# dhg14n9/Light-path-tracer

Hardware: AMD Instinct MI355X
Metric: Mrays/s (higher is better)
Workload: dtype f32

## Files before the change

### include/ltrace.h

```cpp
#ifndef LTRACE_H
#define LTRACE_H

#include <stddef.h>
#include <stdint.h>

#ifdef __cplusplus
extern "C" {
#endif

#define LT_VERSION 200

#define LT_OK 0
#define LT_ERR_INVALID_ARG (-1)
#define LT_ERR_HIP (-2)
#define LT_ERR_NO_DEVICE (-3)
#define LT_ERR_UNSUPPORTED (-4)

#define LT_METRIC_SCHWARZSCHILD 0
#define LT_METRIC_KERR 1

#define LT_INTEGRATOR_DP45 0
#define LT_INTEGRATOR_RK4 1
#define LT_INTEGRATOR_DP45_EXACT 2

// ... 81 lines not shown
                        int8_t *out_status, uint32_t *out_rhs_evals);

int lt_trace_batch_kerr(double M, double a, double r_obs, const double *alphas, const double *thetas,
                        double theta_obs, double lambda_max, const uint8_t *axis_refines,
                        int integrator, int precision, int schedule, int64_t n, double *out_fa,
                        int64_t *out_w, int8_t *out_status, uint32_t *out_rhs_evals);

int lt_trace_batch_kerr_general_probe(double M, double a, double r_obs, const double *alphas, const double *thetas,
                                      double theta_obs, double lambda_max, const uint8_t *axis_refines, int precision,
                                      int64_t n, double *out_fa, int64_t *out_w, int8_t *out_status,
                                      uint32_t *out_rhs_evals);

int lt_set_eq_streak(int on);

int lt_set_unit_streak(int on);

int lt_sincos_q1_probe(uint32_t bits_lo, uint32_t bits_hi, uint64_t out[4], float band[2]);

int lt_kerr_rhs_probe(double M, double a, const double *states, const double *p_phi, int64_t n,
                      int precision, double *out);

int lt_kerr_rhs_form_probe(double M, double a, const double *states, const double *p_phi, int64_t n, int precision,
                           int form, double *out);

int lt_kerr_step_probe(double M, double a, const double *states, const double *p_phi, const uint8_t *refine,
                       const double *h, int64_t n, int precision, int form, double *out_states, double *out_min_r,
                       double *out_max_d, double *out_cs);


int lt_dp45_attempt_probe(double M, double a, double r_obs, double lambda_max, const double *states, const double *p_phi,
// ... 388 lines not shown
```

### light-path-tracer_amd/csrc/lt_api.hip

```cpp
#include "../../include/ltrace.h"
#include "lt_kernels.hpp"
#include "lt_disk.hpp"
#include "lt_disk_images.hpp"
#include "lt_hit_time.hpp"
#include "lt_hotspot.hpp"
#include "lt_polarization.hpp"
#include "lt_aa.hpp"
#include "lt_aa_adaptive.hpp"
#include "lt_hotspot_aa.hpp"
#include "lt_diskmap.hpp"
#include "lt_spectrum.hpp"
#include "lt_visibility.hpp"
#include "lt_visibility_stokes.hpp"
#ifdef LT_PROBES
#include "lt_probe.hpp"
#endif
#include "lt_dense.hpp"

#include <algorithm>
#include <array>
#include <atomic>
#include <cmath>
#include <cstdarg>
#include <cstdio>
// ... 1 lines not shown
#include <cstdlib>
#include <mutex>
#include <type_traits>
#include <utility>
#include <vector>

#ifndef LT_BUILD_ID
#define LT_BUILD_ID "unversioned"
#endif

using namespace lt;

namespace lt {
extern template __global__ void k_kerr_direct<float, Rk4<float>>(KerrConsts<float>, const typename Vec4<float>::type *__restrict__,
                                                                 typename Vec4<float>::type *__restrict__, typename Vec4<float>::type *__restrict__,
                                                                 int64_t, uint32_t, uint4 *__restrict__, uint64_t *__restrict__, unsigned long long *__restrict__);
}

static thread_local char g_err[512] = "";

static int fail(int code, const char *fmt, ...)
{
    va_list ap;
    va_start(ap, fmt);
    vsnprintf(g_err, sizeof(g_err), fmt, ap);
    va_end(ap);
    return code;
}

#define HIP_TRY(expr)                                                                             \
    do {                                                                                          \
// ... 58 lines not shown
    Grow dev;
    Grow dense;
    Grow blocks;
    Grow disk_img;
    Grow disk_time;
    Grow disk_mom;
    Grow hotspot;
    Grow spectrum;
    Grow visibility;
    std::vector<int32_t> blocks_host;
    EventQuad own{};
    bool own_ok = false;
    std::vector<EventQuad> aa_events;
    Grow aa_list;
    Grow aa_scratch;
};

struct Ctx {
    std::vector<StreamSlot *> slots;
    std::vector<EventQuad> pending;
    std::vector<EventQuad> pool;
};

static int slot_events(StreamSlot *sl)
{
    if (sl->own_ok) return LT_OK;
    int made = 0;
    for (auto &e : sl->own.e) {
        if (hipEventCreate(&e) != hipSuccess) break;
        ++made;
    }
    if (made != (int)(sizeof(sl->own.e) / sizeof(sl->own.e[0]))) {
        for (int j = 0; j < made; ++j) (void)hipEventDestroy(sl->own.e[j]);
        return fail(LT_ERR_HIP, "hipEventCreate failed");
    }
    sl->own_ok = true;
    return LT_OK;
}

static std::mutex g_mu;
static Ctx g_ctx[64];
struct MultiStream { int dev, idx; hipStream_t s; };
static std::vector<MultiStream> g_multi_streams;

static int cur_ctx(Ctx **out)
{
    int dev = 0;
    HIP_TRY(hipGetDevice(&dev));
    if (dev < 0 || dev >= 64) return fail(LT_ERR_INVALID_ARG, "device index %d out of range", dev);
    *out = &g_ctx[dev];
    return LT_OK;
// ... 29 lines not shown
    return LT_OK;
}

static void release(Grow &g)
{
    if (g.p) (void)hipFree(g.p);
    g.p = nullptr;
    g.bytes = 0;
}

static void destroy_slot(StreamSlot *sl)
{
    for (Grow *g : {&sl->ws, &sl->dev, &sl->dense, &sl->blocks, &sl->disk_img, &sl->disk_time, &sl->disk_mom, &sl->hotspot, &sl->spectrum, &sl->visibility, &sl->aa_list, &sl->aa_scratch}) release(*g);
    if (sl->own_ok) for (auto &e : sl->own.e) (void)hipEventDestroy(e);
    for (auto &q : sl->aa_events) for (auto &e : q.e) (void)hipEventDestroy(e);
    delete sl;
}

constexpr size_t WS_CTRL_BYTES = 256 + (size_t)STAT_SLOTS * 8 * sizeof(unsigned long long);
struct Workspace {
    unsigned long long *head, *partials;
    char *records;
    size_t n_q;
    template <typename T> typename Vec4<T>::type *ic() const { return (typename Vec4<T>::type *)records; }
    template <typename T> typename Vec4<T>::type *fin0() const { return ic<T>() + n_q; }
    template <typename T> typename Vec4<T>::type *fin1() const { return ic<T>() + 2 * n_q; }
};

template <typename F> static auto with_precision(int precision, F f) { return precision == 32 ? f(float{}) : f(double{}); }
static size_t elem_size(int precision) { return precision == 32 ? sizeof(float) : sizeof(double); }

static int get_workspace(hipStream_t stream, size_t n_q, size_t elem, Workspace *w, StreamSlot **slot = nullptr,
                         IcKey *held = nullptr)
{
    StreamSlot *sl;
    int rc = get_slot(stream, &sl);
    if (rc) return rc;
    if (slot) *slot = sl;
    {
        std::lock_guard<std::mutex> lk(g_mu);
        if (held) *held = sl->ic_key;
        sl->ic_key.valid = false;
    }
    size_t vec = 4 * elem;
    const void *before = sl->ws.p;
    const size_t bytes_before = sl->ws.bytes;
    if ((rc = grow(sl->ws, WS_CTRL_BYTES + 3 * n_q * vec, stream))) return rc;
    if (held && sl->ws.bytes != bytes_before) held->valid = false;
    if (sl->ws.p != before) HIP_TRY(hipMemsetAsync(sl->ws.p, 0, WS_CTRL_BYTES, stream));
    char *base = (char *)sl->ws.p;
    w->head = (unsigned long long *)base;
    w->partials = (unsigned long long *)(base + 256);
    w->records = base + WS_CTRL_BYTES;
    w->n_q = n_q;
    return LT_OK;
}

struct Carver {
    size_t off = 0;
    size_t take(size_t bytes) { size_t o = off; off += (bytes + 255) & ~(size_t)255; return o; }
};

static int env_int(const char *name, int dflt)
{
    const char *e = getenv(name);
    return e ? atoi(e) : dflt;
// ... 27 lines not shown
static bool unit_streak_enabled()
{
    int v = g_unit_streak.load(std::memory_order_relaxed);
    if (v < 0) {
        v = env_int("LT_UNIT_STREAK", 1) != 0;
        int unset = -1;
        if (!g_unit_streak.compare_exchange_strong(unset, v)) v = unset;
    }
    return v != 0;
}
extern "C" int lt_set_unit_streak(int on)
{
    const int before = unit_streak_enabled();
    g_unit_streak.store(on != 0);
    return before;
}

static uint64_t g_ic_hits = 0, g_ic_misses = 0;
extern "C" void lt_ic_reuse_counts(uint64_t *hits, uint64_t *misses)
{
    std::lock_guard<std::mutex> lk(g_mu);
    if (hits) *hits = g_ic_hits;
    if (misses) *misses = g_ic_misses;
}

static int cu_count(int *out)
{
    static int cached[64];
    int dev = 0;
    HIP_TRY(hipGetDevice(&dev));
// ... 349 lines not shown
    return t;
}

template <typename T, typename Go> static int with_integrator(const lt_opts &o, int long_rk4, Go go)
{
    const bool exact = o.integrator == LT_INTEGRATOR_DP45_EXACT;
    const bool dp45 = o.integrator == LT_INTEGRATOR_DP45 || exact;
    if (dp45 && sizeof(T) != 8) return fail(LT_ERR_UNSUPPORTED, "DP45 needs precision 64");
    if constexpr (sizeof(T) == 8) {
        if (exact) return go(IntegTag<Dp45<T, true>>{}, long_rk4 / 3);
        if (dp45) return go(IntegTag<Dp45<T>>{}, long_rk4 / 3);
    }
    return go(IntegTag<Rk4<T>>{}, long_rk4);
}

template <typename T, typename Kernels, typename Launch>
static int launch_direct(const lt_opts &o, const Workspace &w, int64_t n_q, hipStream_t s, int block, Launch launch)
{
    const DirectTuning &tune = direct_tuning();
    return with_integrator<T>(o, tune.long_iters, [&](auto integ, int long_it) -> int {
        constexpr auto kernel = Kernels::template kernel<typename decltype(integ)::type>;
        unsigned grid = (unsigned)((n_q + block - 1) / block);
        unsigned long long *head = nullptr;
        const int slots = tune.persist && block == 64 ? resident_slots<kernel>() : 0;
        if (slots > 0 && (unsigned)slots < grid) { grid = (unsigned)slots; head = w.head; }
        if (head) HIP_TRY(hipMemsetAsync(head, 0, sizeof(unsigned long long), s));
        launch(kernel, grid, (uint32_t)long_it, head);
        HIP_TRY(hipGetLastError());
        return LT_OK;
    });
}

template <typename T>
static int launch_integrate(const MetricConsts &mc, const lt_opts &o, double lambda_max, const Workspace &w,
                            int64_t n_q, hipStream_t s, uint64_t *kstats)
{
    int rc;
    unsigned grid = (unsigned)((n_q + 255) / 256);
    if (mc.kind == LT_METRIC_SCHWARZSCHILD) {
        SchwConsts<T> k = make_schw<T>(mc, o.phi_max, o.h_max);
        k_schw_rk4_direct<T><<<grid, 256, 0, s>>>(k, w.ic<T>(), w.fin0<T>(), w.fin1<T>(), n_q);
    } else {
        KerrConsts<T> k = make_kerr<T>(mc, lambda_max, o.h_max);
        StampDump sd;
        if (o.schedule == LT_SCHED_DIRECT) {
            static const int k2_block = [] { int b = env_int("LT_K2_BLOCK", 64);
                                             return (b == 64 || b == 128 || b == 256) ? b : 64; }();
            if ((rc = sd.begin((size_t)(n_q / 64)))) return rc;
            rc = launch_direct<T, PlainKernels<T>>(o, w, n_q, s, k2_block, [&](auto kernel, unsigned kgrid, uint32_t long_iters, unsigned long long *head) {
                kernel<<<kgrid, k2_block, 0, s>>>(k, w.ic<T>(), w.fin0<T>(), w.fin1<T>(), n_q, long_iters, sd.dev, kstats, head);
            });
            if (rc) return rc;
        } else {
            int cus;
            if ((rc = cu_count(&cus))) return rc;
            static const int bpc = env_int("LT_Q_BPC", sizeof(T) == 4 ? 8 : 3);
            static const int chunk = env_int("LT_Q_CHUNK", 64);
            static const int refill_min = env_int("LT_Q_REFILL", 4);
            static const int long_steps = env_int("LT_Q_LONG", 600);
            unsigned qgrid = (unsigned)(cus * bpc);
            if (qgrid > grid) qgrid = grid;
            rc = with_integrator<T>(o, long_steps, [&](auto integ, int long_it) -> int {
                HIP_TRY(hipMemsetAsync(w.head, 0, sizeof(unsigned long long), s));
                if (int brc = sd.begin((size_t)qgrid * 4)) return brc;
                k_kerr_queue<T, typename decltype(integ)::type><<<qgrid, 256, 0, s>>>(k, w.ic<T>(), w.fin0<T>(), w.fin1<T>(), (uint64_t)n_q, w.head,
// ... 101 lines not shown
            return launch_integrate_disk<decltype(t)>(mc, o, lambda_max, w, n_q, s, kstats, *disk, recs);
        });
    return with_precision(o.precision, [&](auto t) { return launch_integrate<decltype(t)>(mc, o, lambda_max, w, n_q, s, kstats); });
}

template <typename Launch> static void launch_epilogue_rows(const CamConsts &c, const lt_opts &o, const FrameOut &fo, Launch launch)
{
    const bool has_bg = fo.bg != nullptr && (fo.rgb || fo.rgba);
    const dim3 ge((unsigned)((c.W + EPILOGUE_BLOCK - 1) / EPILOGUE_BLOCK), (unsigned)c.rows_local);
    with_precision(o.precision, [&](auto t) {
        if (has_bg) launch(t, std::true_type{}, ge);
        else launch(t, std::false_type{}, ge);
    });
}

static int launch_epilogue_frame(const CamConsts &c, const MetricConsts &mc, const lt_opts &o, const Workspace &w,
                                 const FrameOut &fo, uint64_t *d_stats, hipStream_t s)
{
    if (o.bg_sampling == LT_BG_LDS_TILES && fo.bg && (fo.rgb || fo.rgba)) {
        const unsigned gp = (unsigned)((int64_t)((c.W + 15) / 16) * ((c.rows_local + 15) / 16));
        with_precision(o.precision, [&](auto t) {
            using T = decltype(t);
            k_epilogue_frame_lds<T><<<gp, 256, 0, s>>>(c, mc, w.fin0<T>(), w.fin1<T>(), fo);
        });
    } else {
        launch_epilogue_rows(c, o, fo, [&](auto t, auto bg, dim3 ge) {
            using T = decltype(t);
            k_epilogue_frame<T, decltype(bg)::value><<<ge, EPILOGUE_BLOCK, 0, s>>>(c, mc, w.fin0<T>(), w.fin1<T>(), fo);
        });
    }
    if (d_stats) k_stats_reduce<<<1, STAT_SLOTS, 0, s>>>(w.partials, (unsigned long long *)d_stats, LT_STAT_BG_TILES_LDS, LT_STAT_BG_TILES_GLOBAL);
    HIP_TRY(hipGetLastError());
    return LT_OK;
}

static bool camera_pinhole(const lt_camera *cam, double axis_refine_frac, CamConsts *c)
{
    memset(c, 0, sizeof(*c));
    c->W = cam->width; c->H = cam->height;
    c->half_W = c->W / 2.0; c->half_H = c->H / 2.0;
    c->fx = (c->W / 2.0) / tan(cam->hfov / 2);
    c->fy = (c->H / 2.0) / tan(cam->vfov / 2);
    bool front;
    psi_frame(cam->psi_y, cam->psi_x, c->d, c->ex, c->ey, &front);
    if (front) {
// ... 8 lines not shown
static int make_camera(const lt_camera *cam, int kind, const lt_opts &o, const MetricConsts &mc, const std::vector<int32_t> &owned,
                       int64_t rows_owned, bool listed, bool disk, CamConsts *out)
{
    CamConsts &c = *out;
    const bool front = camera_pinhole(cam, o.axis_refine_frac, &c);
    c.row_block = o.row_block; c.n_parts = o.n_parts; c.part = o.part;
    c.rows_local = (int)rows_owned;
    c.loop_around = o.loop_around;
    c.refine_on = front && kind == LT_METRIC_KERR;
    c.use_tb = !disk && o.tb_symmetry && kind == LT_METRIC_KERR &&
               fabs(cam->theta_obs - M_PI / 2) <= 1e-8 + 1e-5 * (M_PI / 2) && fabs(cam->psi_y) <= 1e-8;
    if (c.use_tb && (o.n_parts != 1 || listed)) return fail(LT_ERR_UNSUPPORTED, "tb_symmetry needs n_parts == 1 and no block_owner table");
    c.trace_rows = c.use_tb ? (c.H + 1) / 2 : c.rows_local;
    c.tiles_x = (c.W + 7) / 8;
    if (c.rows_local <= 0) return LT_OK;
    if (c.rows_local > 65535)
        return fail(LT_ERR_UNSUPPORTED, "a partition of %d rows exceeds the epilogue's launch grid (65535 rows): split it (n_parts)", c.rows_local);
    const int tiles_y = (c.trace_rows + 7) / 8;
    c.tiles_y = tiles_y;
    if (!front || kind != LT_METRIC_KERR) return LT_OK;
    double a = mc.a, M_ = mc.M;
    double b_max = 3.0 * sqrt(3.0) * M_;
    if (a != 0.0) {
        double aa = fabs(a);
        double r_ph = 2.0 * M_ * (1.0 + cos(2.0 / 3.0 * acos(aa / M_)));
        double Dl = r_ph * r_ph - 2.0 * M_ * r_ph + aa * aa;
        double xi = (r_ph * r_ph + aa * aa) / aa - 2.0 * r_ph * Dl / (aa * (r_ph - M_));
        if (fabs(xi) > b_max) b_max = fabs(xi);
    }
    b_max = 1.05 * b_max + 0.3 * M_;
    double f0 = 1.0 - 2.0 * M_ / cam->r_obs;
// ... 55 lines not shown
    if (key.has_blocks) key.blocks = owned;
    key.kind = mc.kind; key.obs_ok = mc.obs_ok;
    const double mkey[15] = {mc.M, mc.a, mc.r_obs, mc.theta_obs, mc.R_S, mc.obs_sin_th, mc.obs_cos2, mc.obs_sin2, mc.obs_sqrt_Sigma,
                             mc.obs_sqrt_Delta, mc.obs_g_tt, mc.obs_g_tphi, mc.obs_g_rr, mc.obs_g_thth, mc.obs_g_phiphi};
    memcpy(key.metric, mkey, sizeof(mkey));
    key.elem = elem; key.n_q = n_q;
    return key;
}

struct KeyGuard {
    StreamSlot *sl;
    bool ok = false;
    ~KeyGuard() { if (ok) return; std::lock_guard<std::mutex> lk(g_mu); sl->ic_key.valid = false; }
};

static int render_dev_impl(const lt_camera *cam, const lt_metric *metric, const lt_opts *opts, const float *d_bg,
                           int32_t bg_channels, float *d_fa, uint16_t *d_w, int8_t *d_status, uint32_t *d_steps,
                           float *d_rgb, uint8_t *d_rgba, uint64_t *d_stats, const EventQuad *own_events,
                           const DiskParams *disk = nullptr, const AaBand *aa = nullptr)
{
    int rc = require_device();
    if (rc) return rc;
    if (!cam || !metric || !opts) return fail(LT_ERR_INVALID_ARG, "null camera / metric / opts");
    if (cam->width <= 0 || cam->height <= 0) return fail(LT_ERR_INVALID_ARG, "empty frame %dx%d", cam->width, cam->height);
    if (d_bg && bg_channels != 1 && bg_channels != 3) return fail(LT_ERR_INVALID_ARG, "bg_channels must be 1 or 3");
    lt_opts o = *opts;
    if ((rc = check_opts(metric, &o))) return rc;
    MetricConsts mc;
    if ((rc = make_metric(metric, cam->r_obs, cam->theta_obs, o.h_max, &mc))) return rc;
    count_evals(o.integrator, &mc);
// ... 22 lines not shown

    const size_t elem = elem_size(o.precision);
    Workspace w;
    StreamSlot *slot;
    IcKey held;
    if ((rc = get_workspace(s, (size_t)n_q, elem, &w, &slot, &held))) return rc;
    IcKey key = make_ic_key(c, owned, mc, elem, n_q);
    const bool reuse = ic_reuse_enabled() && key.same(held);
    KeyGuard guard{slot};
    DiskRecordsBuf recs;
    if ((rc = get_disk_records(s, n_q, elem, disk, &recs))) return rc;
    Timer tm;
    if ((rc = tm.begin(o.timing != 0, own_events))) return rc;
    FrameOut fo{d_bg, bg_channels, d_fa, d_w, d_status, d_steps, d_rgb, d_rgba, d_stats ? (uint64_t *)w.partials : nullptr};

    if ((rc = tm.mark(0, s))) return rc;
    if (!reuse && (rc = launch_prologue_camera(c, mc, o, w, n_q, s))) return rc;
    {
        std::lock_guard<std::mutex> lk(g_mu);
        slot->ic_key = std::move(key);
        ++(reuse ? g_ic_hits : g_ic_misses);
    }
    if ((rc = tm.mark(1, s))) return rc;
    if ((rc = launch_integrate_any(mc, o, lambda_max, w, n_q, s, d_stats, disk, recs))) return rc;
    if ((rc = tm.mark(2, s))) return rc;
    if (aa) rc = launch_epilogue_aa(c, mc, o, w, fo, d_stats, s, disk, recs, *aa);
    else if (!disk) rc = launch_epilogue_frame(c, mc, o, w, fo, d_stats, s);
    else if (disk->max_images) rc = launch_epilogue_disk_images(c, mc, o, w, fo, d_stats, s, *disk, recs);
    else rc = launch_epilogue_disk(c, mc, o, w, fo, d_stats, s, *disk);
    if (rc) return rc;
    if ((rc = tm.mark(3, s))) return rc;
    tm.finish();
    guard.ok = true;
    return LT_OK;
}

extern "C" int lt_render_dev(const lt_camera *cam, const lt_metric *metric, const lt_opts *opts, const float *d_bg,
                             int32_t bg_channels, float *d_fa, uint16_t *d_w, int8_t *d_status, uint32_t *d_steps,
// ... 822 lines not shown
```

### light-path-tracer_amd/csrc/lt_k2_lone.hip

```cpp
#include <hip/hip_runtime.h>
#include <cstdint>
#include "../../include/ltrace.h"
#define LT_KERNEL_TEMPLATES_ONLY
#include "lt_kernels.hpp"

namespace lt {
template __global__ void k_kerr_direct<float, Rk4<float>>(KerrConsts<float>, const typename Vec4<float>::type *__restrict__,
                                                          typename Vec4<float>::type *__restrict__, typename Vec4<float>::type *__restrict__,
                                                          int64_t, uint32_t, uint4 *__restrict__, uint64_t *__restrict__, unsigned long long *__restrict__);
}
```

### light-path-tracer_amd/csrc/lt_kernels.hpp

```cpp
#pragma once
#include "lt_device.hpp"
#include "lt_dp45.hpp"

namespace lt {

template <typename T> struct Vec4;
template <> struct Vec4<float> { using type = float4; };
template <> struct Vec4<double> { using type = double4; };

constexpr int FLAG_OK = 1, FLAG_REFINE = 2, FLAG_PAD = 4;

struct CamConsts {
    int W, H;
    int rows_local;
    int trace_rows;
    int use_tb;
    int tiles_x, tiles_y;
    int strip_x0, strip_x1;
    int hot_x0, hot_x1, hot_y0, hot_y1;
    int row_block, n_parts, part;
    const int32_t *block_list;
    int loop_around;
    double half_W, half_H, fx, fy;
    double d[3], ex[3], ey[3];
// ... 305 lines not shown
    __device__ __forceinline__ void begin_tile(Lane &, const KerrConsts<T> &) {}
    __device__ __forceinline__ void bind(Lane &, const KerrConsts<T> &, const RayConsts<T> &) {}
    __device__ __forceinline__ const KerrConsts<T> &streak_consts(const Lane &, const KerrConsts<T> &k) const { return k; }
    __device__ __forceinline__ int advance(Lane &, const KerrConsts<T> &k, const RayConsts<T> &rc, typename Integ::State &st, int64_t, bool)
    {
        return Integ::advance(k, rc, st);
    }
    __device__ __forceinline__ void stored(Lane &, int64_t) {}
};

template <typename T, typename Integ, typename Step>
__device__ __forceinline__ void direct_tiles(const KerrConsts<T> &k_in, Step step, const typename Vec4<T>::type *__restrict__ ic,
                                             typename Vec4<T>::type *__restrict__ fin0,
                                             typename Vec4<T>::type *__restrict__ fin1, int64_t n_q, uint32_t long_iters,
                                             uint4 *__restrict__ stamps, uint64_t *__restrict__ kstats,
                                             unsigned long long *__restrict__ head)
{
    KerrConsts<T> k = k_in;
    pin_consts(k);
    const int lane = (int)(threadIdx.x & 63u);
    int64_t tile = (int64_t)blockIdx.x * (blockDim.x >> 6) + (threadIdx.x >> 6);
    for (;;) {
    if (head) {
        unsigned long long w = 0;
        if (lane == 0) w = atomicAdd(head, 1ull);
        tile = (int64_t)(((uint64_t)__builtin_amdgcn_readfirstlane((uint32_t)(w >> 32)) << 32) |
                         (uint64_t)__builtin_amdgcn_readfirstlane((uint32_t)w));
    }
    const int64_t q = tile * 64 + lane;
    if (q >= n_q) return;
    uint64_t t0 = stamps ? wave_clock() : 0, c0 = stamps ? __builtin_amdgcn_s_memtime() : 0;
    WaveMeter meter;
    meter.begin(kstats, tile);
    typename Vec4<T>::type rec = ic[q];
    int flags = (int)rec.w;
    typename Integ::State st;
    st.y.r = k.r_obs; st.y.th = k.theta_obs; st.y.ph = T(0); st.y.pr = rec.x; st.y.pth = rec.y;
    st.steps = 0;
    int ev = (flags & FLAG_PAD) ? EV_PAD : EV_INVALID;
    uint32_t wave_iters = 0;
    uint32_t eq_iters = 0;
    bool raised = false;
// ... 57 lines not shown
        store_fin<T>(fin0, fin1, q, st.y.r, st.y.th, st.y.ph, st.y.pr, st.y.pth, rec.z, ev, steps);
        step.stored(ls, q);
    }
    meter.end(kstats, wave_iters, eq_iters);
    if (stamps) write_stamp(stamps, tile, t0, steps, c0);
    if (!head) return;
    if (__builtin_amdgcn_ballot_w64(raised)) __builtin_amdgcn_s_setprio(0);
    }
}

template <typename T, typename Integ>
__global__ void __launch_bounds__(256, Integ::MIN_WAVES_PER_SIMD) k_kerr_direct(KerrConsts<T> k_in, const typename Vec4<T>::type *__restrict__ ic,
                                                         typename Vec4<T>::type *__restrict__ fin0,
                                                         typename Vec4<T>::type *__restrict__ fin1, int64_t n_q,
                                                         uint32_t long_iters, uint4 *__restrict__ stamps,
                                                         uint64_t *__restrict__ kstats, unsigned long long *__restrict__ head)
{
    direct_tiles<T, Integ>(k_in, PlainStep<T, Integ>{}, ic, fin0, fin1, n_q, long_iters, stamps, kstats, head);
}

template <typename T, typename Integ>
__global__ void __launch_bounds__(256, Integ::MIN_WAVES_PER_SIMD) k_kerr_queue(KerrConsts<T> k_in, const typename Vec4<T>::type *__restrict__ ic,
                                                        typename Vec4<T>::type *__restrict__ fin0,
                                                        typename Vec4<T>::type *__restrict__ fin1, uint64_t n_q,
                                                        unsigned long long *__restrict__ head, uint32_t chunk,
                                                        uint32_t refill_min, uint32_t long_steps,
                                                        uint4 *__restrict__ stamps, uint64_t *__restrict__ kstats)
{
    uint64_t t0 = stamps ? wave_clock() : 0, c0 = stamps ? __builtin_amdgcn_s_memtime() : 0;
    const int64_t wave_id = (int64_t)blockIdx.x * (blockDim.x >> 6) + (threadIdx.x >> 6);
    WaveMeter meter;
    meter.begin(kstats, wave_id);
    KerrConsts<T> k = k_in;
// ... 317 lines not shown

__device__ __forceinline__ void store_rgba(const FrameOut &o, int64_t p, const float *rgb, int nch)
{
    uchar4 px;
    px.x = (uint8_t)(rgb[0] * 255.0f);
    px.y = (uint8_t)(rgb[nch == 1 ? 0 : 1] * 255.0f);
    px.z = (uint8_t)(rgb[nch == 1 ? 0 : 2] * 255.0f);
    px.w = 255;
    reinterpret_cast<uchar4 *>(o.rgba)[p] = px;
}

constexpr int EPILOGUE_BLOCK = 512;
template <typename T, bool HAS_BG>
__global__ void __launch_bounds__(EPILOGUE_BLOCK) k_epilogue_frame(CamConsts c, MetricConsts m,
                                                                   const typename Vec4<T>::type *__restrict__ fin0,
                                                                   const typename Vec4<T>::type *__restrict__ fin1, FrameOut o)
{
    const int lrow = (int)blockIdx.y, ix = (int)(blockIdx.x * EPILOGUE_BLOCK + threadIdx.x);
    const int64_t p = (int64_t)lrow * c.W + ix;
    StatAcc acc;
    if (ix < c.W) {
        int src_row = lrow;
        if (c.use_tb && lrow >= c.H - c.H / 2) src_row = c.H - 1 - lrow;
        RayResult res;
        load_result<T>(m, fin0, fin1, pixel_to_q(c, ix, src_row), res);
        if (src_row == lrow) acc.add(res);
        float fa32 = (res.status == 1) ? (float)res.fa : __builtin_nanf("");
        long long wl = res.n_half < 0 ? 0 : (res.n_half > 65535 ? 65535 : res.n_half);
        if (o.fa) o.fa[p] = fa32;
        if (o.w) o.w[p] = (uint16_t)wl;
        if (o.status) o.status[p] = (int8_t)res.status;
        if (o.steps) o.steps[p] = res.steps;
        if (o.rgb || o.rgba) {
// ... 552 lines not shown
```

### light-path-tracer_amd/ltrace.py

```python
import ctypes as C
import os

import numpy as np

_HERE = os.path.dirname(os.path.abspath(__file__))
LIB_PATH = os.environ.get("LTRACE_LIB", os.path.join(_HERE, "lib", "libltrace_hip.so"))

OK, ERR_INVALID_ARG, ERR_HIP, ERR_NO_DEVICE, ERR_UNSUPPORTED = 0, -1, -2, -3, -4
METRIC_SCHWARZSCHILD, METRIC_KERR = 0, 1
INTEGRATOR_DP45, INTEGRATOR_RK4, INTEGRATOR_DP45_EXACT = 0, 1, 2
SCHED_DIRECT, SCHED_QUEUE = 0, 1
STAT_RAYS, STAT_STEPS, STAT_RHS_EVALS, STAT_ESCAPED, STAT_CAPTURED, STAT_INVALID = range(6)
STAT_WAVE_ITERS, STAT_WAVES, STAT_CLK_CYCLES, STAT_CLK_TICKS = 6, 7, 8, 9
STAT_BG_TILES_LDS, STAT_BG_TILES_GLOBAL = 10, 11
STAT_DISK = 12
STAT_DISK_HITS = 13
STAT_AA_REFINED = 14
STAT_EQ_ITERS = 15
DISK_MAX_IMAGES = 8
STATUS_DISK = 2
STAT_WORDS = 16

INTEGRATORS = {"dp45": INTEGRATOR_DP45, "rk4": INTEGRATOR_RK4, "dp45_exact": INTEGRATOR_DP45_EXACT}
SCHEDULES = {"direct": SCHED_DIRECT, "queue": SCHED_QUEUE}
# ... 121 lines not shown
    "lt_dp45_controller_probe": (C.c_int, [C.c_int, C.c_void_p, C.c_void_p, C.c_int64, C.c_void_p, C.c_void_p]),
    "lt_ic_probe": (C.c_int, [C.c_int] + [C.c_double] * 4 + [C.c_void_p] * 3 + [C.c_int64, C.c_int, C.c_void_p]),
    "lt_rk4_advance_probe": (C.c_int, [C.c_double] * 5 + [C.c_void_p] * 6 + [C.c_int64, C.c_int, C.c_int] + [C.c_void_p] * 3),
    "lt_schw_trace_probe": (C.c_int, [C.c_double] * 4 + [C.c_void_p] * 2 + [C.c_int64, C.c_int] + [C.c_void_p] * 4),
    "lt_extract_probe": (C.c_int, [C.c_int, C.c_double, C.c_double, C.c_double, C.c_int, C.c_void_p, C.c_void_p, C.c_int64, C.c_int]
                         + [C.c_void_p] * 4),
    "lt_math32_probe": (C.c_int, [C.c_int, C.c_uint32, C.c_uint32, C.c_void_p, C.c_int, C.c_void_p]),
    "lt_math64_probe": (C.c_int, [C.c_int, C.c_void_p, C.c_int64, C.c_void_p]),
    "lt_disk_crossing_probe": (C.c_int, [C.POINTER(Metric), C.c_double, C.c_double] + [C.c_void_p] * 5 + [C.c_int64, C.c_int]
                               + [C.c_void_p] * 3),
    "lt_disk_advance_probe": (C.c_int, [C.POINTER(Metric)] + [C.c_double] * 5 + [C.c_int, C.c_int] + [C.c_void_p] * 6 + [C.c_int64]
                              + [C.c_void_p] * 5),
    "lt_disk_shade_probe": (C.c_int, [C.POINTER(Metric), C.c_double, C.c_double, C.c_double, C.c_void_p, C.c_int64] + [C.c_void_p] * 3),
    "lt_set_eq_streak": (C.c_int, [C.c_int]),
    "lt_set_unit_streak": (C.c_int, [C.c_int]),
    "lt_sincos_q1_probe": (C.c_int, [C.c_uint32, C.c_uint32, C.c_void_p, C.c_void_p]),
    "lt_local_rows": (C.c_int64, [C.c_int32, C.c_int32, C.c_int32, C.c_int32]),
    "lt_global_row": (C.c_int64, [C.c_int64, C.c_int32, C.c_int32, C.c_int32]),
    "lt_render_dev": (C.c_int, [C.POINTER(Camera), C.POINTER(Metric), C.POINTER(Opts), C.c_void_p, C.c_int32,
                                C.c_void_p, C.c_void_p, C.c_void_p, C.c_void_p, C.c_void_p, C.c_void_p, C.c_void_p]),
    "lt_render": (C.c_int, [C.POINTER(Camera), C.POINTER(Metric), C.POINTER(Opts), C.c_void_p, C.c_int32,
                            C.c_void_p, C.c_void_p, C.c_void_p, C.c_void_p, C.c_void_p, C.c_void_p,
                            C.POINTER(Stats)]),
    "lt_scatter_rows_dev": (C.c_int, [C.c_void_p, C.c_void_p, C.c_int32, C.c_int32, C.c_int32, C.c_int32,
                                      C.c_int32, C.c_int32, C.c_void_p]),
    "lt_scatter_rows_indexed_dev": (C.c_int, [C.c_void_p, C.c_void_p, C.c_void_p, C.c_int64, C.c_int64, C.c_int64, C.c_void_p]),
    "lt_timing_collect": (C.c_int, [_dp, _dp, _dp, C.POINTER(C.c_int32)]),
    "lt_ic_reuse_counts": (None, [C.POINTER(C.c_uint64), C.POINTER(C.c_uint64)]),
    "lt_pixel_angles": (C.c_int, [C.POINTER(Camera), C.c_double, C.c_void_p, C.c_void_p, C.c_void_p]),
    "lt_shade": (C.c_int, [C.POINTER(Camera), C.c_int32, C.c_void_p, C.c_int32, C.c_void_p, C.c_void_p,
# ... 446 lines not shown
def math64_probe(which, x):
    xx = np.ascontiguousarray(x, dtype=np.float64).ravel()
    out = np.empty((xx.size, 2))
    _check(load().lt_math64_probe(MATH64_WHICH[which], _np_ptr(xx), xx.size, _np_ptr(out)))
    return out


def set_eq_streak(on):
    return bool(load().lt_set_eq_streak(int(bool(on))))


def set_unit_streak(on):
    return bool(load().lt_set_unit_streak(int(bool(on))))


def sincos_q1_probe(bits_lo, bits_hi):
    out = np.zeros(4, dtype=np.uint64)
    band = np.zeros(2, dtype=np.float32)
    _check(load().lt_sincos_q1_probe(int(bits_lo), int(bits_hi), _np_ptr(out), _np_ptr(band)))
    return dict(compared=int(out[0]), differing=int(out[1]), outside_k1=int(out[2]), first_differing_bits=int(out[3]),
                band=(float(band[0]), float(band[1])))


def local_rows(height, row_block, n_parts, part):
    return int(load().lt_local_rows(height, row_block, n_parts, part))


def global_rows(height, row_block, n_parts, part):
    n = local_rows(height, row_block, n_parts, part)
    lib = load()
# ... 968 lines not shown
```

Baseline: 1592.

## Split direct-schedule integration into two tile queues to overlap epilogue

Splits the Kerr direct-schedule tile queue into a main part and a tail of bottom tile rows. The tail is integrated on a low-priority side stream with its own persistent head counter. The epilogue for the finished top rows runs on the main stream while the tail integrates, and a joining event gates the remaining epilogue rows. This is meant to fill idle compute slots at the end of integration and hide part of the epilogue, at the cost of extra stream and event overhead and two persistent kernels competing for compute units.

After: 1624 (median of 6 runs). 1.02x the previous value.

```diff
diff --git a/include/ltrace.h b/include/ltrace.h
--- a/include/ltrace.h
+++ b/include/ltrace.h
@@ -119,6 +119,13 @@
 int lt_set_eq_streak(int on);
 
 int lt_set_unit_streak(int on);
+
+int lt_set_tail_split(int tile_rows);
+
+void lt_tail_split_counts(uint64_t *split, uint64_t *whole);
+
+int lt_tail_split_plan(int32_t tiles_x, int32_t tiles_y, int32_t strip_x0, int32_t strip_x1, int32_t hot_y1, int32_t slots,
+                       int32_t request, int32_t *ty_split, int64_t *pos_split);
 
 int lt_sincos_q1_probe(uint32_t bits_lo, uint32_t bits_hi, uint64_t out[4], float band[2]);
 
diff --git a/light-path-tracer_amd/csrc/lt_api.hip b/light-path-tracer_amd/csrc/lt_api.hip
--- a/light-path-tracer_amd/csrc/lt_api.hip
+++ b/light-path-tracer_amd/csrc/lt_api.hip
@@ -39,7 +39,8 @@
 namespace lt {
 extern template __global__ void k_kerr_direct<float, Rk4<float>>(KerrConsts<float>, const typename Vec4<float>::type *__restrict__,
                                                                  typename Vec4<float>::type *__restrict__, typename Vec4<float>::type *__restrict__,
-                                                                 int64_t, uint32_t, uint4 *__restrict__, uint64_t *__restrict__, unsigned long long *__restrict__);
+                                                                 int64_t, uint32_t, uint4 *__restrict__, uint64_t *__restrict__, unsigned long long *__restrict__,
+                                                                 int64_t);
 }
 
 static thread_local char g_err[512] = "";
@@ -128,6 +129,8 @@
     std::vector<EventQuad> aa_events;
     Grow aa_list;
     Grow aa_scratch;
+    hipStream_t side = nullptr;
+    hipEvent_t fork = nullptr, join = nullptr;
 };
 
 struct Ctx {
@@ -149,6 +152,26 @@
         return fail(LT_ERR_HIP, "hipEventCreate failed");
     }
     sl->own_ok = true;
+    return LT_OK;
+}
+
+static int slot_side(StreamSlot *sl)
+{
+    if (sl->side) return LT_OK;
+    int least = 0, greatest = 0;
+    HIP_TRY(hipDeviceGetStreamPriorityRange(&least, &greatest));
+    hipStream_t side = nullptr;
+    hipEvent_t fork = nullptr, join = nullptr;
+    hipError_t e = hipStreamCreateWithPriority(&side, hipStreamNonBlocking, least);
+    if (e == hipSuccess) e = hipEventCreateWithFlags(&fork, hipEventDisableTiming);
+    if (e == hipSuccess) e = hipEventCreateWithFlags(&join, hipEventDisableTiming);
+    if (e != hipSuccess) {
+        if (join) (void)hipEventDestroy(join);
+        if (fork) (void)hipEventDestroy(fork);
+        if (side) (void)hipStreamDestroy(side);
+        return fail(LT_ERR_HIP, "creating the side stream of a slot failed: %s", hipGetErrorString(e));
+    }
+    sl->side = side; sl->fork = fork; sl->join = join;
     return LT_OK;
 }
 
@@ -208,12 +231,18 @@
     for (Grow *g : {&sl->ws, &sl->dev, &sl->dense, &sl->blocks, &sl->disk_img, &sl->disk_time, &sl->disk_mom, &sl->hotspot, &sl->spectrum, &sl->visibility, &sl->aa_list, &sl->aa_scratch}) release(*g);
     if (sl->own_ok) for (auto &e : sl->own.e) (void)hipEventDestroy(e);
     for (auto &q : sl->aa_events) for (auto &e : q.e) (void)hipEventDestroy(e);
+    if (sl->side) {
+        (void)hipStreamSynchronize(sl->side);
+        (void)hipEventDestroy(sl->fork);
+        (void)hipEventDestroy(sl->join);
+        (void)hipStreamDestroy(sl->side);
+    }
     delete sl;
 }
 
 constexpr size_t WS_CTRL_BYTES = 256 + (size_t)STAT_SLOTS * 8 * sizeof(unsigned long long);
 struct Workspace {
-    unsigned long long *head, *partials;
+    unsigned long long *head, *head_b, *partials;
     char *records;
     size_t n_q;
     template <typename T> typename Vec4<T>::type *ic() const { return (typename Vec4<T>::type *)records; }
@@ -244,6 +273,7 @@
     if (sl->ws.p != before) HIP_TRY(hipMemsetAsync(sl->ws.p, 0, WS_CTRL_BYTES, stream));
     char *base = (char *)sl->ws.p;
     w->head = (unsigned long long *)base;
+    w->head_b = (unsigned long long *)(base + 128);
     w->partials = (unsigned long long *)(base + 256);
     w->records = base + WS_CTRL_BYTES;
     w->n_q = n_q;
@@ -301,6 +331,70 @@
     const int before = unit_streak_enabled();
     g_unit_streak.store(on != 0);
     return before;
+}
+
+constexpr int TAIL_SPLIT_DEFAULT = -1;
+static std::atomic<int> g_tail_split{INT32_MIN};
+static int tail_split_request()
+{
+    int v = g_tail_split.load(std::memory_order_relaxed);
+    if (v == INT32_MIN) {
+        v = env_int("LT_TAIL_SPLIT", TAIL_SPLIT_DEFAULT);
+        if (v < -1) v = -1;
+        int unset = INT32_MIN;
+        if (!g_tail_split.compare_exchange_strong(unset, v)) v = unset;
+    }
+    return v;
+}
+extern "C" int lt_set_tail_split(int tile_rows)
+{
+    const int before = tail_split_request();
+    g_tail_split.store(tile_rows < -1 ? -1 : tile_rows);
+    return before;
+}
+
+constexpr int TAIL_SPLIT_FILLS_NUM = 1, TAIL_SPLIT_FILLS_DEN = 1, TAIL_SPLIT_MIN_FILLS_A = 1;
+static bool tail_split_plan(int tiles_x, int tiles_y, int strip_w, int hot_y1, int slots, int request, int *ty_split,
+                            int64_t *pos_split)
+{
+    const int64_t n_tiles = (int64_t)tiles_x * tiles_y;
+    *ty_split = tiles_y;
+    *pos_split = n_tiles;
+    const int64_t cw = (int64_t)tiles_x - strip_w;
+    int64_t avail = (int64_t)tiles_y - hot_y1;
+    if (request == 0 || cw <= 0 || avail <= 0) return false;
+    int64_t rows_b;
+    if (request > 0) {
+        if (avail * cw >= n_tiles) --avail;
+        rows_b = request < avail ? request : avail;
+    } else {
+        if (slots <= 0) return false;
+        rows_b = ((int64_t)TAIL_SPLIT_FILLS_NUM * slots + TAIL_SPLIT_FILLS_DEN * cw - 1) / (TAIL_SPLIT_FILLS_DEN * cw);
+        if (rows_b > avail || n_tiles - rows_b * cw < (int64_t)TAIL_SPLIT_MIN_FILLS_A * slots) return false;
+    }
+    if (rows_b <= 0) return false;
+    *ty_split = (int)(tiles_y - rows_b);
+    *pos_split = n_tiles - rows_b * cw;
+    return true;
+}
+extern "C" int lt_tail_split_plan(int32_t tiles_x, int32_t tiles_y, int32_t strip_x0, int32_t strip_x1, int32_t hot_y1, int32_t slots,
+                                  int32_t request, int32_t *ty_split, int64_t *pos_split)
+{
+    int ty = 0;
+    int64_t pos = 0;
+    if (tiles_x <= 0 || tiles_y <= 0 || strip_x0 < 0 || strip_x1 < strip_x0 || strip_x1 > tiles_x || hot_y1 < 0 || hot_y1 > tiles_y) return -1;
+    const bool on = tail_split_plan(tiles_x, tiles_y, strip_x1 - strip_x0, hot_y1, slots, request, &ty, &pos);
+    if (ty_split) *ty_split = ty;
+    if (pos_split) *pos_split = pos;
+    return on ? 1 : 0;
+}
+
+static uint64_t g_split_frames = 0, g_whole_frames = 0;
+extern "C" void lt_tail_split_counts(uint64_t *split, uint64_t *whole)
+{
+    std::lock_guard<std::mutex> lk(g_mu);
+    if (split) *split = g_split_frames;
+    if (whole) *whole = g_whole_frames;
 }
 
 static uint64_t g_ic_hits = 0, g_ic_misses = 0;
@@ -680,26 +774,54 @@
     return go(IntegTag<Rk4<T>>{}, long_rk4);
 }
 
+struct QueuePart {
+    int64_t tile0, n_tiles;
+    unsigned long long *head;
+    int64_t q_end() const { return (tile0 + n_tiles) * 64; }
+};
+
 template <typename T, typename Kernels, typename Launch>
-static int launch_direct(const lt_opts &o, const Workspace &w, int64_t n_q, hipStream_t s, int block, Launch launch)
+static int launch_direct(const lt_opts &o, const QueuePart &part, hipStream_t s, int block, Launch launch)
 {
     const DirectTuning &tune = direct_tuning();
     return with_integrator<T>(o, tune.long_iters, [&](auto integ, int long_it) -> int {
         constexpr auto kernel = Kernels::template kernel<typename decltype(integ)::type>;
-        unsigned grid = (unsigned)((n_q + block - 1) / block);
+        unsigned grid = (unsigned)((part.n_tiles * 64 + block - 1) / block);
         unsigned long long *head = nullptr;
         const int slots = tune.persist && block == 64 ? resident_slots<kernel>() : 0;
-        if (slots > 0 && (unsigned)slots < grid) { grid = (unsigned)slots; head = w.head; }
+        if (slots > 0 && (unsigned)slots < grid) { grid = (unsigned)slots; head = part.head; }
         if (head) HIP_TRY(hipMemsetAsync(head, 0, sizeof(unsigned long long), s));
         launch(kernel, grid, (uint32_t)long_it, head);
         HIP_TRY(hipGetLastError());
         return LT_OK;
     });
 }
+template <typename T, typename Kernels, typename Launch>
+static int launch_direct(const lt_opts &o, const Workspace &w, int64_t n_q, hipStream_t s, int block, Launch launch)
+{
+    return launch_direct<T, Kernels>(o, QueuePart{0, n_q / 64, w.head}, s, block, launch);
+}
+
+static int k2_block()
+{
+    static const int b = [] { int v = env_int("LT_K2_BLOCK", 64); return (v == 64 || v == 128 || v == 256) ? v : 64; }();
+    return b;
+}
+
+template <typename T> static int direct_slots(const lt_opts &o)
+{
+    int slots = 0;
+    if (!direct_tuning().persist || k2_block() != 64) return 0;
+    (void)with_integrator<T>(o, 0, [&](auto integ, int) -> int {
+        slots = resident_slots<PlainKernels<T>::template kernel<typename decltype(integ)::type>>();
+        return LT_OK;
+    });
+    return slots;
+}
 
 template <typename T>
 static int launch_integrate(const MetricConsts &mc, const lt_opts &o, double lambda_max, const Workspace &w,
-                            int64_t n_q, hipStream_t s, uint64_t *kstats)
+                            int64_t n_q, hipStream_t s, uint64_t *kstats, const QueuePart *part = nullptr)
 {
     int rc;
     unsigned grid = (unsigned)((n_q + 255) / 256);
@@ -710,11 +832,10 @@
         KerrConsts<T> k = make_kerr<T>(mc, lambda_max, o.h_max);
         StampDump sd;
         if (o.schedule == LT_SCHED_DIRECT) {
-            static const int k2_block = [] { int b = env_int("LT_K2_BLOCK", 64);
-                                             return (b == 64 || b == 128 || b == 256) ? b : 64; }();
+            const QueuePart qp = part ? *part : QueuePart{0, n_q / 64, w.head};
             if ((rc = sd.begin((size_t)(n_q / 64)))) return rc;
-            rc = launch_direct<T, PlainKernels<T>>(o, w, n_q, s, k2_block, [&](auto kernel, unsigned kgrid, uint32_t long_iters, unsigned long long *head) {
-                kernel<<<kgrid, k2_block, 0, s>>>(k, w.ic<T>(), w.fin0<T>(), w.fin1<T>(), n_q, long_iters, sd.dev, kstats, head);
+            rc = launch_direct<T, PlainKernels<T>>(o, qp, s, k2_block(), [&](auto kernel, unsigned kgrid, uint32_t long_iters, unsigned long long *head) {
+                kernel<<<kgrid, k2_block(), 0, s>>>(k, w.ic<T>(), w.fin0<T>(), w.fin1<T>(), qp.q_end(), long_iters, sd.dev, kstats, head, qp.tile0);
             });
             if (rc) return rc;
         } else {
@@ -846,21 +967,43 @@
     });
 }
 
+template <typename Launch>
+static void launch_epilogue_rows(const CamConsts &c, const lt_opts &o, const FrameOut &fo, int row0, int row1, Launch launch)
+{
+    const bool has_bg = fo.bg != nullptr && (fo.rgb || fo.rgba);
+    with_precision(o.precision, [&](auto t) {
+        for (int r = row0; r < row1; r += std::min(row1 - r, 65535)) {
+            const dim3 ge((unsigned)((c.W + EPILOGUE_BLOCK - 1) / EPILOGUE_BLOCK), (unsigned)std::min(row1 - r, 65535));
+            if (has_bg) launch(t, std::true_type{}, ge, r);
+            else launch(t, std::false_type{}, ge, r);
+        }
+    });
+}
+
+static bool epilogue_is_lds(const lt_opts &o, const FrameOut &fo) { return o.bg_sampling == LT_BG_LDS_TILES && fo.bg && (fo.rgb || fo.rgba); }
+
+static int launch_epilogue_frame_rows(const CamConsts &c, const MetricConsts &mc, const lt_opts &o, const Workspace &w,
+                                      const FrameOut &fo, hipStream_t s, int row0, int row1)
+{
+    launch_epilogue_rows(c, o, fo, row0, row1, [&](auto t, auto bg, dim3 ge, int r0) {
+        using T = decltype(t);
+        k_epilogue_frame<T, decltype(bg)::value><<<ge, EPILOGUE_BLOCK, 0, s>>>(c, mc, w.fin0<T>(), w.fin1<T>(), fo, r0);
+    });
+    HIP_TRY(hipGetLastError());
+    return LT_OK;
+}
+
 static int launch_epilogue_frame(const CamConsts &c, const MetricConsts &mc, const lt_opts &o, const Workspace &w,
-                                 const FrameOut &fo, uint64_t *d_stats, hipStream_t s)
-{
-    if (o.bg_sampling == LT_BG_LDS_TILES && fo.bg && (fo.rgb || fo.rgba)) {
+                                 const FrameOut &fo, uint64_t *d_stats, hipStream_t s, int row0 = 0)
+{
+    if (epilogue_is_lds(o, fo)) {
         const unsigned gp = (unsigned)((int64_t)((c.W + 15) / 16) * ((c.rows_local + 15) / 16));
         with_precision(o.precision, [&](auto t) {
             using T = decltype(t);
             k_epilogue_frame_lds<T><<<gp, 256, 0, s>>>(c, mc, w.fin0<T>(), w.fin1<T>(), fo);
         });
-    } else {
-        launch_epilogue_rows(c, o, fo, [&](auto t, auto bg, dim3 ge) {
-            using T = decltype(t);
-            k_epilogue_frame<T, decltype(bg)::value><<<ge, EPILOGUE_BLOCK, 0, s>>>(c, mc, w.fin0<T>(), w.fin1<T>(), fo);
-        });
-    }
+    } else if (int rc = launch_epilogue_frame_rows(c, mc, o, w, fo, s, row0, c.rows_local))
+        return rc;
     if (d_stats) k_stats_reduce<<<1, STAT_SLOTS, 0, s>>>(w.partials, (unsigned long long *)d_stats, LT_STAT_BG_TILES_LDS, LT_STAT_BG_TILES_GLOBAL);
     HIP_TRY(hipGetLastError());
     return LT_OK;
@@ -899,7 +1042,7 @@
     c.trace_rows = c.use_tb ? (c.H + 1) / 2 : c.rows_local;
     c.tiles_x = (c.W + 7) / 8;
     if (c.rows_local <= 0) return LT_OK;
-    if (c.rows_local > 65535)
+    if (disk && c.rows_local > 65535)
         return fail(LT_ERR_UNSUPPORTED, "a partition of %d rows exceeds the epilogue's launch grid (65535 rows): split it (n_parts)", c.rows_local);
     const int tiles_y = (c.trace_rows + 7) / 8;
     c.tiles_y = tiles_y;
@@ -985,6 +1128,20 @@
     ~KeyGuard() { if (ok) return; std::lock_guard<std::mutex> lk(g_mu); sl->ic_key.valid = false; }
 };
 
+struct SideJoin {
+    StreamSlot *sl;
+    hipStream_t s;
+    bool recorded = false, waited = false;
+    int record() { HIP_TRY(hipEventRecord(sl->join, sl->side)); recorded = true; return LT_OK; }
+    int wait() { HIP_TRY(hipStreamWaitEvent(s, sl->join, 0)); waited = true; return LT_OK; }
+    ~SideJoin()
+    {
+        if (waited) return;
+        if ((!recorded && hipEventRecord(sl->join, sl->side) != hipSuccess) || hipStreamWaitEvent(s, sl->join, 0) != hipSuccess)
+            (void)hipStreamSynchronize(sl->side);
+    }
+};
+
 static int render_dev_impl(const lt_camera *cam, const lt_metric *metric, const lt_opts *opts, const float *d_bg,
                            int32_t bg_channels, float *d_fa, uint16_t *d_w, int8_t *d_status, uint32_t *d_steps,
                            float *d_rgb, uint8_t *d_rgba, uint64_t *d_stats, const EventQuad *own_events,
@@ -1037,14 +1194,55 @@
     if ((rc = tm.begin(o.timing != 0, own_events))) return rc;
     FrameOut fo{d_bg, bg_channels, d_fa, d_w, d_status, d_steps, d_rgb, d_rgba, d_stats ? (uint64_t *)w.partials : nullptr};
 
+    int ty_split = c.tiles_y;
+    int64_t pos_split = n_q / 64;
+    bool split = false;
+    const int split_request = tail_split_request();
+    if (split_request != 0 && !disk && !aa && mc.kind == LT_METRIC_KERR && o.schedule == LT_SCHED_DIRECT && !c.use_tb &&
+        !epilogue_is_lds(o, fo) && !getenv("LT_STAMPS_FILE")) {
+        hipStreamCaptureStatus capturing = hipStreamCaptureStatusNone;
+        if (hipStreamIsCapturing(s, &capturing) != hipSuccess) {
+            (void)hipGetLastError();
+            capturing = hipStreamCaptureStatusActive;
+        }
+        if (capturing == hipStreamCaptureStatusNone) {
+            const int slots = with_precision(o.precision, [&](auto t) { return direct_slots<decltype(t)>(o); });
+            split = tail_split_plan(c.tiles_x, c.tiles_y, c.strip_x1 - c.strip_x0, c.hot_y1, slots, split_request, &ty_split, &pos_split);
+        }
+    }
+
     if ((rc = tm.mark(0, s))) return rc;
     if (!reuse && (rc = launch_prologue_camera(c, mc, o, w, n_q, s))) return rc;
     {
         std::lock_guard<std::mutex> lk(g_mu);
         slot->ic_key = std::move(key);
         ++(reuse ? g_ic_hits : g_ic_misses);
+        ++(split ? g_split_frames : g_whole_frames);
     }
     if ((rc = tm.mark(1, s))) return rc;
+    if (split) {
+        const int64_t n_tiles = n_q / 64;
+        const QueuePart part_a{0, pos_split, w.head}, part_b{pos_split, n_tiles - pos_split, w.head_b};
+        const int rows_a = std::min(ty_split * 8, c.rows_local);
+        if ((rc = slot_side(slot))) return rc;
+        HIP_TRY(hipEventRecord(slot->fork, s));
+        SideJoin sj{slot, s};
+        auto integrate = [&](const QueuePart &part, hipStream_t on) {
+            return with_precision(o.precision, [&](auto t) { return launch_integrate<decltype(t)>(mc, o, lambda_max, w, n_q, on, d_stats, &part); });
+        };
+        if ((rc = integrate(part_a, s))) return rc;
+        HIP_TRY(hipStreamWaitEvent(slot->side, slot->fork, 0));
+        if ((rc = integrate(part_b, slot->side))) return rc;
+        if ((rc = sj.record())) return rc;
+        if (rows_a > 0 && (rc = launch_epilogue_frame_rows(c, mc, o, w, fo, s, 0, rows_a))) return rc;
+        if ((rc = sj.wait())) return rc;
+        if ((rc = tm.mark(2, s))) return rc;
+        if ((rc = launch_epilogue_frame(c, mc, o, w, fo, d_stats, s, rows_a))) return rc;
+        if ((rc = tm.mark(3, s))) return rc;
+        tm.finish();
+        guard.ok = true;
+        return LT_OK;
+    }
     if ((rc = launch_integrate_any(mc, o, lambda_max, w, n_q, s, d_stats, disk, recs))) return rc;
     if ((rc = tm.mark(2, s))) return rc;
     if (aa) rc = launch_epilogue_aa(c, mc, o, w, fo, d_stats, s, disk, recs, *aa);
diff --git a/light-path-tracer_amd/csrc/lt_k2_lone.hip b/light-path-tracer_amd/csrc/lt_k2_lone.hip
--- a/light-path-tracer_amd/csrc/lt_k2_lone.hip
+++ b/light-path-tracer_amd/csrc/lt_k2_lone.hip
@@ -7,5 +7,6 @@
 namespace lt {
 template __global__ void k_kerr_direct<float, Rk4<float>>(KerrConsts<float>, const typename Vec4<float>::type *__restrict__,
                                                           typename Vec4<float>::type *__restrict__, typename Vec4<float>::type *__restrict__,
-                                                          int64_t, uint32_t, uint4 *__restrict__, uint64_t *__restrict__, unsigned long long *__restrict__);
+                                                          int64_t, uint32_t, uint4 *__restrict__, uint64_t *__restrict__, unsigned long long *__restrict__,
+                                                          int64_t);
 }
diff --git a/light-path-tracer_amd/csrc/lt_kernels.hpp b/light-path-tracer_amd/csrc/lt_kernels.hpp
--- a/light-path-tracer_amd/csrc/lt_kernels.hpp
+++ b/light-path-tracer_amd/csrc/lt_kernels.hpp
@@ -343,18 +343,18 @@
                                              typename Vec4<T>::type *__restrict__ fin0,
                                              typename Vec4<T>::type *__restrict__ fin1, int64_t n_q, uint32_t long_iters,
                                              uint4 *__restrict__ stamps, uint64_t *__restrict__ kstats,
-                                             unsigned long long *__restrict__ head)
+                                             unsigned long long *__restrict__ head, int64_t tile0 = 0)
 {
     KerrConsts<T> k = k_in;
     pin_consts(k);
     const int lane = (int)(threadIdx.x & 63u);
-    int64_t tile = (int64_t)blockIdx.x * (blockDim.x >> 6) + (threadIdx.x >> 6);
+    int64_t tile = tile0 + (int64_t)blockIdx.x * (blockDim.x >> 6) + (threadIdx.x >> 6);
     for (;;) {
     if (head) {
         unsigned long long w = 0;
         if (lane == 0) w = atomicAdd(head, 1ull);
-        tile = (int64_t)(((uint64_t)__builtin_amdgcn_readfirstlane((uint32_t)(w >> 32)) << 32) |
-                         (uint64_t)__builtin_amdgcn_readfirstlane((uint32_t)w));
+        tile = tile0 + (int64_t)(((uint64_t)__builtin_amdgcn_readfirstlane((uint32_t)(w >> 32)) << 32) |
+                                 (uint64_t)__builtin_amdgcn_readfirstlane((uint32_t)w));
     }
     const int64_t q = tile * 64 + lane;
     if (q >= n_q) return;
@@ -442,9 +442,10 @@
                                                          typename Vec4<T>::type *__restrict__ fin0,
                                                          typename Vec4<T>::type *__restrict__ fin1, int64_t n_q,
                                                          uint32_t long_iters, uint4 *__restrict__ stamps,
-                                                         uint64_t *__restrict__ kstats, unsigned long long *__restrict__ head)
-{
-    direct_tiles<T, Integ>(k_in, PlainStep<T, Integ>{}, ic, fin0, fin1, n_q, long_iters, stamps, kstats, head);
+                                                         uint64_t *__restrict__ kstats, unsigned long long *__restrict__ head,
+                                                         int64_t tile0)
+{
+    direct_tiles<T, Integ>(k_in, PlainStep<T, Integ>{}, ic, fin0, fin1, n_q, long_iters, stamps, kstats, head, tile0);
 }
 
 template <typename T, typename Integ>
@@ -792,9 +793,10 @@
 template <typename T, bool HAS_BG>
 __global__ void __launch_bounds__(EPILOGUE_BLOCK) k_epilogue_frame(CamConsts c, MetricConsts m,
                                                                    const typename Vec4<T>::type *__restrict__ fin0,
-                                                                   const typename Vec4<T>::type *__restrict__ fin1, FrameOut o)
-{
-    const int lrow = (int)blockIdx.y, ix = (int)(blockIdx.x * EPILOGUE_BLOCK + threadIdx.x);
+                                                                   const typename Vec4<T>::type *__restrict__ fin1, FrameOut o,
+                                                                   int row0)
+{
+    const int lrow = row0 + (int)blockIdx.y, ix = (int)(blockIdx.x * EPILOGUE_BLOCK + threadIdx.x);
     const int64_t p = (int64_t)lrow * c.W + ix;
     StatAcc acc;
     if (ix < c.W) {
diff --git a/light-path-tracer_amd/ltrace.py b/light-path-tracer_amd/ltrace.py
--- a/light-path-tracer_amd/ltrace.py
+++ b/light-path-tracer_amd/ltrace.py
@@ -159,6 +159,9 @@
     "lt_disk_shade_probe": (C.c_int, [C.POINTER(Metric), C.c_double, C.c_double, C.c_double, C.c_void_p, C.c_int64] + [C.c_void_p] * 3),
     "lt_set_eq_streak": (C.c_int, [C.c_int]),
     "lt_set_unit_streak": (C.c_int, [C.c_int]),
+    "lt_set_tail_split": (C.c_int, [C.c_int]),
+    "lt_tail_split_counts": (None, [C.POINTER(C.c_uint64), C.POINTER(C.c_uint64)]),
+    "lt_tail_split_plan": (C.c_int, [C.c_int32] * 7 + [C.POINTER(C.c_int32), C.POINTER(C.c_int64)]),
     "lt_sincos_q1_probe": (C.c_int, [C.c_uint32, C.c_uint32, C.c_void_p, C.c_void_p]),
     "lt_local_rows": (C.c_int64, [C.c_int32, C.c_int32, C.c_int32, C.c_int32]),
     "lt_global_row": (C.c_int64, [C.c_int64, C.c_int32, C.c_int32, C.c_int32]),
@@ -635,6 +638,24 @@
     return bool(load().lt_set_unit_streak(int(bool(on))))
 
 
+def set_tail_split(tile_rows):
+    return int(load().lt_set_tail_split(int(tile_rows)))
+
+
+def tail_split_counts():
+    a, b = C.c_uint64(), C.c_uint64()
+    load().lt_tail_split_counts(C.byref(a), C.byref(b))
+    return int(a.value), int(b.value)
+
+
+def tail_split_plan(tiles_x, tiles_y, strip_x0, strip_x1, hot_y1, slots, request):
+    ty, pos = C.c_int32(), C.c_int64()
+    r = load().lt_tail_split_plan(tiles_x, tiles_y, strip_x0, strip_x1, hot_y1, slots, request, C.byref(ty), C.byref(pos))
+    if r < 0:
+        raise LtraceError(ERR_INVALID_ARG, "lt_tail_split_plan: the arguments describe no frame")
+    return bool(r), int(ty.value), int(pos.value)
+
+
 def sincos_q1_probe(bits_lo, bits_hi):
     out = np.zeros(4, dtype=np.uint64)
     band = np.zeros(2, dtype=np.float32)
```
